# fernandezdaniel/MOBOCMF

Measured on AMD Instinct MI355X. Metric: ELBO steps/sec (MFDGP d=8 M=512 N=8192 S=8), higher is better.
Workload: dtype f64

## Files before the change

mobocmf_amd/csrc/elementwise.hip:

```cpp
#include "common.h"

#define LOG_2PI 1.8378770664093454835606594728112

__device__ __forceinline__ double wave_sum(double v) {
    v += __shfl_xor(v, 1);
    v += __shfl_xor(v, 2);
    v += __shfl_xor(v, 4);
    v += __shfl_xor(v, 8);
    v += __shfl_xor(v, 16);
    v += __shfl_xor(v, 32);
    return v;
}

__device__ __forceinline__ double block_sum(double v, double* sh) {
    v = wave_sum(v);
    const int lane = threadIdx.x & 63, wave = threadIdx.x >> 6;
    __syncthreads();
    if (lane == 0) sh[wave] = v;
    __syncthreads();
    double t = 0.0;
    if (threadIdx.x == 0)
        for (int w = 0; w < (int)(blockDim.x >> 6); ++w) t += sh[w];
    return t;
}
// ... 12 lines not shown

#define GRID1(n) dim3((unsigned)(((n) + 255) / 256)), dim3(256)
#define CHECK_LAUNCH() (hipGetLastError() == hipSuccess ? MOBOCMF_OK : MOBOCMF_HIP_ERROR)

__global__ void zero32_kernel(uint32_t* p, int64_t n) {
    int64_t i = (int64_t)blockIdx.x * blockDim.x + threadIdx.x;
    if (i < n) p[i] = 0u;
}
int launch_zero32(void* ptr, int64_t nwords, hipStream_t s) {
    if (nwords <= 0) return MOBOCMF_OK;
    hipLaunchKernelGGL(zero32_kernel, GRID1(nwords), 0, s, (uint32_t*)ptr, nwords);
    return CHECK_LAUNCH();
}
#define GRIDZ(n, nz) dim3((unsigned)(((n) + 255) / 256), 1, (unsigned)(nz)), dim3(256)
struct ScalZ { const double* p[MAX_ZL]; };
__global__ void zero32_z_kernel(uint32_t* p, int64_t n, int64_t zs_words) {
    int64_t i = (int64_t)blockIdx.x * blockDim.x + threadIdx.x;
    if (i < n) p[blockIdx.z * zs_words + i] = 0u;
}
int launch_zero32_z(void* ptr, int64_t nwords, int nz, int64_t zs_bytes, hipStream_t s) {
    if (nwords <= 0) return MOBOCMF_OK;
    hipLaunchKernelGGL(zero32_z_kernel, GRIDZ(nwords, nz), 0, s, (uint32_t*)ptr, nwords, zs_bytes / 4);
    return CHECK_LAUNCH();
}

__global__ void pad_tril_kernel(const double* src, int64_t lds, int M, double* dst, int Mp) {
    int64_t idx = (int64_t)blockIdx.x * blockDim.x + threadIdx.x;
    if (idx >= (int64_t)Mp * Mp) return;
    int i = (int)(idx / Mp), j = (int)(idx % Mp);
    dst[idx] = (i < M && j <= i) ? src[(int64_t)i * lds + j] : 0.0;
}
int launch_pad_tril(const double* src, int64_t lds, int M, double* dst, int Mp, hipStream_t s) {
    hipLaunchKernelGGL(pad_tril_kernel, GRID1((int64_t)Mp * Mp), 0, s, src, lds, M, dst, Mp);
    return CHECK_LAUNCH();
}

__global__ void pad_vec_kernel(const double* src, int64_t n, double* dst, int64_t np) {
    int64_t i = (int64_t)blockIdx.x * blockDim.x + threadIdx.x;
    if (i < np) dst[i] = (src && i < n) ? src[i] : 0.0;
}
int launch_pad_vec(const double* src, int64_t n, double* dst, int64_t np, hipStream_t s) {
    hipLaunchKernelGGL(pad_vec_kernel, GRID1(np), 0, s, src, n, dst, np);
    return CHECK_LAUNCH();
}

struct PadZ { const double* LS[MAX_ZL]; const double* m[MAX_ZL]; };
__global__ void pad_params_z_kernel(PadZ t, int M, double* LSp, double* mp, int Mp, int64_t zs) {
    int64_t idx = (int64_t)blockIdx.x * blockDim.x + threadIdx.x;
    if (idx >= (int64_t)Mp * Mp) return;
    const int z = blockIdx.z;
    int i = (int)(idx / Mp), j = (int)(idx % Mp);
    LSp[z * zs + idx] = (i < M && j <= i) ? t.LS[z][(int64_t)i * M + j] : 0.0;
    if (idx < Mp) mp[z * zs + idx] = idx < M ? t.m[z][idx] : 0.0;
}
int launch_pad_params_z(const double* const* LS, const double* const* m, int M, double* LSp, double* mp, int Mp, int nz,
                        int64_t zs, hipStream_t s) {
    PadZ t = {};
    for (int z = 0; z < nz; ++z) { t.LS[z] = LS[z]; t.m[z] = m[z]; }
    hipLaunchKernelGGL(pad_params_z_kernel, GRIDZ((int64_t)Mp * Mp, nz), 0, s, t, M, LSp, mp, Mp, zs);
    return CHECK_LAUNCH();
}

__global__ void transpose_kernel(const double* in, int64_t ldi, double* out, int64_t ldo, int64_t rows, int64_t cols,
                                 int64_t zs) {
    __shared__ double t[32][33];
    in += blockIdx.z * zs;
    out += blockIdx.z * zs;
    int64_t c = (int64_t)blockIdx.x * 32 + threadIdx.x, r0 = (int64_t)blockIdx.y * 32;
    for (int k = threadIdx.y; k < 32; k += 8)
        if (r0 + k < rows && c < cols) t[k][threadIdx.x] = in[(r0 + k) * ldi + c];
    __syncthreads();
    int64_t r = r0 + threadIdx.x, c0 = (int64_t)blockIdx.x * 32;
    for (int k = threadIdx.y; k < 32; k += 8)
        if (c0 + k < cols && r < rows) out[(c0 + k) * ldo + r] = t[threadIdx.x][k];
}
int launch_transpose_z(const double* in, int64_t ldi, double* out, int64_t ldo, int64_t rows, int64_t cols, int nz,
                       int64_t zs, hipStream_t s) {
    dim3 grid((unsigned)((cols + 31) / 32), (unsigned)((rows + 31) / 32), (unsigned)nz);
    hipLaunchKernelGGL(transpose_kernel, grid, dim3(32, 8), 0, s, in, ldi, out, ldo, rows, cols, zs);
    return CHECK_LAUNCH();
}
__global__ void transpose_pad_z_kernel(const double* in, double* out, int Mp, int64_t zs, PadZ t, int M, double* LSp, double* mp) {
    __shared__ double tl[32][33];
    const int z = blockIdx.z;
    in += z * zs; out += z * zs;
    const int64_t c = (int64_t)blockIdx.x * 32 + threadIdx.x, r0 = (int64_t)blockIdx.y * 32;
    for (int k = threadIdx.y; k < 32; k += 8) {
        const int64_t i = r0 + k;
        tl[k][threadIdx.x] = in[i * Mp + c];
        LSp[z * zs + i * Mp + c] = (i < M && c <= i) ? t.LS[z][i * M + c] : 0.0;
        if (i == 0) mp[z * zs + c] = c < M ? t.m[z][c] : 0.0;
    }
    __syncthreads();
    const int64_t r = r0 + threadIdx.x, c0 = (int64_t)blockIdx.x * 32;
    for (int k = threadIdx.y; k < 32; k += 8) out[(c0 + k) * Mp + r] = tl[threadIdx.x][k];
}
int launch_transpose_pad_z(const double* in, double* out, int Mp, const double* const* LS, const double* const* m, int M,
                           double* LSp, double* mp, int nz, int64_t zs, hipStream_t s) {
    PadZ t = {};
    for (int z = 0; z < nz; ++z) { t.LS[z] = LS[z]; t.m[z] = m[z]; }
    hipLaunchKernelGGL(transpose_pad_z_kernel, dim3((unsigned)(Mp / 32), (unsigned)(Mp / 32), (unsigned)nz), dim3(32, 8), 0, s, in,
                       out, Mp, zs, t, M, LSp, mp);
    return CHECK_LAUNCH();
}
__global__ void transpose_gemv_z_kernel(const double* in, double* out, int Mp, int64_t zs, const double* Mat, const double* vec,
                                        double* vout) {
    __shared__ double tl[32][33];
    const int z = blockIdx.z;
    in += z * zs; out += z * zs; Mat += z * zs; vec += z * zs; vout += z * zs;
    const int64_t c = (int64_t)blockIdx.x * 32 + threadIdx.x, r0 = (int64_t)blockIdx.y * 32;
    for (int k = threadIdx.y; k < 32; k += 8) tl[k][threadIdx.x] = in[(r0 + k) * Mp + c];
    {
        const int tid = threadIdx.y * 32 + threadIdx.x, wave = tid >> 6, lane = tid & 63;
        const int nblk = gridDim.x * gridDim.y, b = blockIdx.y * gridDim.x + blockIdx.x;
        for (int row = 4 * b + wave; row < Mp; row += 4 * nblk) {
            const double* p = Mat + (int64_t)row * Mp;
            double sacc = 0.0;
            for (int j = lane; j < Mp; j += 64) sacc += p[j] * vec[j];
            sacc = wave_sum(sacc);
            if (lane == 0) vout[row] = sacc;
        }
    }
    __syncthreads();
    const int64_t r = r0 + threadIdx.x, c0 = (int64_t)blockIdx.x * 32;
    for (int k = threadIdx.y; k < 32; k += 8) out[(c0 + k) * Mp + r] = tl[threadIdx.x][k];
}
int launch_transpose_gemv_z(const double* in, double* out, int Mp, const double* Mat, const double* vec, double* vout, int nz,
                            int64_t zs, hipStream_t s) {
    hipLaunchKernelGGL(transpose_gemv_z_kernel, dim3((unsigned)(Mp / 32), (unsigned)(Mp / 32), (unsigned)nz), dim3(32, 8), 0, s, in,
                       out, Mp, zs, Mat, vec, vout);
    return CHECK_LAUNCH();
}
int launch_transpose(const double* in, int64_t ldi, double* out, int64_t ldo, int64_t rows, int64_t cols, hipStream_t s) {
    return launch_transpose_z(in, ldi, out, ldo, rows, cols, 1, 0, s);
}

__global__ void gemv_rows_kernel(const double* Mat, int64_t ld, const double* vec, double* out, int rows, int64_t cols,
                                 double scale, int accumulate, int64_t zs) {
    int row = blockIdx.x * 4 + (threadIdx.x >> 6);
    int lane = threadIdx.x & 63;
    if (row >= rows) return;
    Mat += blockIdx.z * zs; vec += blockIdx.z * zs; out += blockIdx.z * zs;
    const double* p = Mat + (int64_t)row * ld;
    double s = 0.0;
    for (int64_t j = lane; j < cols; j += 64) s += p[j] * vec[j];
    s = wave_sum(s) * scale;
    if (lane == 0) out[row] = accumulate ? out[row] + s : s;
}
int launch_gemv_rows_z(const double* Mat, int64_t ld, const double* vec, double* out, int rows, int64_t cols, double scale,
                       int accumulate, int nz, int64_t zs, hipStream_t s) {
    hipLaunchKernelGGL(gemv_rows_kernel, dim3((rows + 3) / 4, 1, nz), dim3(256), 0, s, Mat, ld, vec, out, rows, cols, scale,
                       accumulate, zs);
    return CHECK_LAUNCH();
}
int launch_gemv_rows(const double* Mat, int64_t ld, const double* vec, double* out, int rows, int64_t cols, double scale,
                     int accumulate, hipStream_t s) {
    return launch_gemv_rows_z(Mat, ld, vec, out, rows, cols, scale, accumulate, 1, 0, s);
}

__global__ void kl_part_kernel(const double* L, const double* LSp, const double* U, const double* a, int M, int Mp,
                               double* part, int64_t zs) {
    __shared__ double sh[4];
    double s = 0.0;
    const int r0 = blockIdx.x * 4;
    L += blockIdx.z * zs; LSp += blockIdx.z * zs; U += blockIdx.z * zs; a += blockIdx.z * zs; part += blockIdx.z * zs;
    for (int rr = 0; rr < 4; ++rr) {
        const int i = r0 + rr;
        if (i >= M) break;
        const double* u = U + (int64_t)i * Mp;
        for (int j = threadIdx.x; j <= i; j += 256) s += u[j] * u[j];
        if (threadIdx.x == 0) {
            double l = L[(int64_t)i * Mp + i], ls = LSp[(int64_t)i * Mp + i];
            s += 2.0 * log(l) - log(ls * ls) + a[i] * a[i];
        }
    }
    s = block_sum(s, sh);
    if (threadIdx.x == 0) part[blockIdx.x] = s;
}
struct KlZ { double* p[MAX_ZL]; };
__global__ void kl_final_kernel(const double* part, int np, int M, KlZ kl, int64_t zs) {
    __shared__ double sh[4];
    double s = 0.0;
    part += blockIdx.x * zs;
    for (int i = threadIdx.x; i < np; i += 256) s += part[i];
    s = block_sum(s, sh);
    if (threadIdx.x == 0) kl.p[blockIdx.x][0] = 0.5 * (s - (double)M);
}
__global__ __launch_bounds__(1024) void kl_one_kernel(const double* L, const double* LSp, const double* U, const double* a, int M,
                                                      int Mp, KlZ kl, int64_t zs) {
    __shared__ double sh[16];
    const int z = blockIdx.x;
    L += z * zs; LSp += z * zs; U += z * zs; a += z * zs;
    double s = 0.0;
    const int total = M * Mp;
#pragma unroll 4
    for (int e = threadIdx.x; e < total; e += 1024) {
        const int i = e / Mp, j = e - i * Mp;
        const double u = U[e];
        s += j <= i ? u * u : 0.0;
    }
    for (int i = threadIdx.x; i < M; i += 1024) {
        const double l = L[(int64_t)i * Mp + i], ls = LSp[(int64_t)i * Mp + i];
        s += 2.0 * log(l) - log(ls * ls) + a[i] * a[i];
    }
    s = wave_sum(s);
    if ((threadIdx.x & 63) == 0) sh[threadIdx.x >> 6] = s;
    __syncthreads();
    if (threadIdx.x == 0) {
        double t = 0.0;
        for (int w = 0; w < 16; ++w) t += sh[w];
        kl.p[z][0] = 0.5 * (t - (double)M);
    }
}
int launch_kl_z(const double* L, const double* LSp, const double* U, const double* a, int M, int Mp, double* const* kl,
                double* part, int nz, int64_t zs, hipStream_t s) {
    if (M <= 128) {
        KlZ kz1 = {};
        for (int z = 0; z < nz; ++z) kz1.p[z] = kl[z];
        hipLaunchKernelGGL(kl_one_kernel, dim3(nz), dim3(1024), 0, s, L, LSp, U, a, M, Mp, kz1, zs);
        return CHECK_LAUNCH();
    }
    const int nb = (M + 3) / 4;
    hipLaunchKernelGGL(kl_part_kernel, dim3(nb, 1, nz), dim3(256), 0, s, L, LSp, U, a, M, Mp, part, zs);
    KlZ kz = {};
    for (int z = 0; z < nz; ++z) kz.p[z] = kl[z];
    hipLaunchKernelGGL(kl_final_kernel, dim3(nz), dim3(256), 0, s, (const double*)part, nb, M, kz, zs);
    return CHECK_LAUNCH();
}
int launch_kl(const double* L, const double* LSp, const double* U, const double* a, int M, int Mp, double* kl,
              double* part, hipStream_t s) {
    double* one[1] = {kl};
    return launch_kl_z(L, LSp, U, a, M, Mp, one, part, 1, 0, s);
}

__global__ void moments_finish_kernel(const double* qpart, const double* mupart, const double* rpart, int nrb,
                                      int64_t Np, int64_t N, const double* knn, int branch, double min_var, double* q,
                                      double* r, double* varraw, double* mean, double* var, int32_t* zero_word) {
    int64_t n = (int64_t)blockIdx.x * blockDim.x + threadIdx.x;
    if (n == 0 && zero_word) zero_word[0] = 0;
    if (n >= Np) return;
    double qs = 0, ms = 0, rs = 0;
    for (int b = 0; b < nrb; ++b) {
        qs += qpart[(int64_t)b * Np + n];
        ms += mupart[(int64_t)b * Np + n];
        rs += rpart[(int64_t)b * Np + n];
    }
    double sres = knn[n] - qs;
    if (!branch && sres < 0.0) sres = 0.0;
    double v = sres + rs;
    q[n] = qs;
    r[n] = rs;
    varraw[n] = v;
    if (n < N) {
        mean[n] = ms;
        var[n] = v < min_var ? min_var : v;
    }
}
int launch_moments_finish(const double* qpart, const double* mupart, const double* rpart, int nrb, int64_t Np, int64_t N,
                          const double* knn, int branch, double min_var, double* q, double* r, double* varraw,
                          double* mean, double* var, int32_t* zero_word, hipStream_t s) {
    hipLaunchKernelGGL(moments_finish_kernel, GRID1(Np), 0, s, qpart, mupart, rpart, nrb, Np, N, knn, branch, min_var, q,
                       r, varraw, mean, var, zero_word);
    return CHECK_LAUNCH();
}

__global__ void moments_bwd_prep_kernel(const double* g_mean, const double* g_var, const double* knn, const double* q,
                                        const double* varraw, int branch, double min_var, int64_t N, int64_t Np,
                                        double* gmu, double* gv, double* gv2, double* cgv, int32_t* nclamped, int32_t* blkact) {
    __shared__ int any_w[4];
    int64_t n = (int64_t)blockIdx.x * blockDim.x + threadIdx.x;
    double gm = 0.0, g = 0.0, c = 0.0;
    if (n < N) {
        gm = g_mean ? g_mean[n] : 0.0;
        g = (g_var && varraw[n] > min_var) ? g_var[n] : 0.0;
        c = (branch || knn[n] - q[n] > 0.0) ? g : 0.0;
        if (c != g) atomicAdd(nclamped, 1);
    }
    if (n < Np) {
        gmu[n] = gm;
        gv[n] = g;
        gv2[n] = 2.0 * g;
        cgv[n] = c;
    }
    if (blkact) {
        const bool any = !(gm == 0.0) || !(g == 0.0);
        const unsigned long long b = __ballot(any);
        if ((threadIdx.x & 63) == 0) any_w[threadIdx.x >> 6] = b != 0ull ? 1 : 0;
        __syncthreads();
        if (threadIdx.x < 2) {
            const int64_t blk = (int64_t)blockIdx.x * 2 + threadIdx.x;
            if (blk * 128 < Np) blkact[blk] = any_w[2 * threadIdx.x] | any_w[2 * threadIdx.x + 1];
        }
    }
}
int launch_moments_bwd_prep(const double* g_mean, const double* g_var, const double* knn, const double* q,
                            const double* varraw, int branch, double min_var, int64_t N, int64_t Np, double* gmu,
                            double* gv, double* gv2, double* cgv, int32_t* nclamped, int zeroed, int32_t* blkact, hipStream_t s) {
    if (!zeroed && launch_zero32(nclamped, 1, s)) return MOBOCMF_HIP_ERROR;
    hipLaunchKernelGGL(moments_bwd_prep_kernel, GRID1(Np), 0, s, g_mean, g_var, knn, q, varraw, branch, min_var, N, Np,
                       gmu, gv, gv2, cgv, nclamped, blkact);
    return CHECK_LAUNCH();
}

__device__ __forceinline__ double slab_sum(const double* p, int64_t slab_stride, int ns) {
    double v = 0.0;
    int z = 0;
    for (; z + 8 <= ns; z += 8) {
        double t[8];
#pragma unroll
        for (int b = 0; b < 8; ++b) t[b] = p[(z + b) * slab_stride];
#pragma unroll
        for (int b = 0; b < 8; ++b) v += t[b];
    }
    for (; z < ns; ++z) v += p[z * slab_stride];
    return v;
}

__global__ void reduce_slabs_sym_kernel(const double* slabs, int64_t slab_stride, int nslab, int nslab_diag, double* out,
                                        int Mp, const int32_t* flag, const double* fallback) {
    int64_t idx = (int64_t)blockIdx.x * blockDim.x + threadIdx.x;
    if (idx >= (int64_t)Mp * Mp) return;
    int i = (int)(idx / Mp), j = (int)(idx % Mp);
    if (flag && *flag == 0) {
        out[idx] = fallback[idx];
        return;
    }
    if (j / TILE > i / TILE) return;
    const double* p = j > i ? slabs + (int64_t)j * Mp + i : slabs + (int64_t)i * Mp + j;
    const int ns = (i / TILE == j / TILE) ? nslab_diag : nslab;
    const double v = slab_sum(p, slab_stride, ns);
    out[idx] = v;
    if (j / TILE < i / TILE) out[(int64_t)j * Mp + i] = v;
}
__global__ void reduce_slabs_sym2_kernel(const double* slabs, const double* slabs2, int64_t slab_stride, int nslab,
                                         int nslab_diag, double* out, double* out2, int Mp, const int32_t* flag) {
    int64_t idx = (int64_t)blockIdx.x * blockDim.x + threadIdx.x;
    if (idx >= (int64_t)Mp * Mp) return;
    int i = (int)(idx / Mp), j = (int)(idx % Mp);
    if (j / TILE > i / TILE) return;
    const int64_t off = j > i ? (int64_t)j * Mp + i : (int64_t)i * Mp + j;
    const int ns = (i / TILE == j / TILE) ? nslab_diag : nslab;
    const double v = slab_sum(slabs + off, slab_stride, ns);
    double v2 = v;
    if (*flag != 0) v2 = slab_sum(slabs2 + off, slab_stride, ns);
    out[idx] = v;
    out2[idx] = v2;
    if (j / TILE < i / TILE) { out[(int64_t)j * Mp + i] = v; out2[(int64_t)j * Mp + i] = v2; }
}
int launch_reduce_slabs_sym2(const double* slabs, const double* slabs2, int64_t slab_stride, int nslab, int nslab_diag,
                             double* out, double* out2, int Mp, const int32_t* flag, hipStream_t s) {
    hipLaunchKernelGGL(reduce_slabs_sym2_kernel, GRID1((int64_t)Mp * Mp), 0, s, slabs, slabs2, slab_stride, nslab, nslab_diag,
                       out, out2, Mp, flag);
    return CHECK_LAUNCH();
}
int launch_reduce_slabs_sym(const double* slabs, int64_t slab_stride, int nslab, int nslab_diag, double* out, int Mp,
                            const int32_t* flag, const double* fallback, hipStream_t s) {
    hipLaunchKernelGGL(reduce_slabs_sym_kernel, GRID1((int64_t)Mp * Mp), 0, s, slabs, slab_stride, nslab, nslab_diag, out, Mp,
                       flag, fallback);
    return CHECK_LAUNCH();
}

__global__ void dutot_y_kernel(const double* G1, const double* G2, const double* Hc, const double* U, const double* da,
                               const double* a, ScalZ gklz, int Mp, double* dU, double* da_tot, double* Y, int64_t zs) {
    __shared__ double tl[32][33];
    const double* gkl = gklz.p[blockIdx.z];
    const double g = gkl ? gkl[0] : 0.0;
    const int64_t zo = blockIdx.z * zs;
    G1 += zo; G2 += zo; Hc += zo; U += zo; da += zo; a += zo; dU += zo; da_tot += zo; Y += zo;
    const int nt = Mp / 32, ti = blockIdx.x / nt, tj = blockIdx.x % nt;
    const int tx = threadIdx.x & 31, ty = threadIdx.x >> 5;
    if (tj <= ti) {
#pragma unroll
        for (int r = ty; r < 32; r += 8) tl[r][tx] = G1[(int64_t)(tj * 32 + r) * Mp + ti * 32 + tx];
    }
    __syncthreads();
#pragma unroll
    for (int r = ty; r < 32; r += 8) {
        const int i = ti * 32 + r, j = tj * 32 + tx;
        const int64_t idx = (int64_t)i * Mp + j;
        const double ai = a[i], aj = a[j], dai = da[i], daj = da[j];
        dU[idx] = j <= i ? 2.0 * tl[tx][r] + g * U[idx] : 0.0;
        Y[idx] = 2.0 * (G2[idx] - Hc[idx]) + ai * daj + (dai + g * ai) * aj;
        if (tj == 0 && tx == 0) da_tot[i] = dai + g * ai;
    }
}
int launch_dutot_y_z(const double* G1, const double* G2, const double* Hc, const double* U, const double* da, const double* a,
                     const double* const* gkl, int Mp, double* dU, double* da_tot, double* Y, int nz, int64_t zs, hipStream_t s) {
    ScalZ t = {};
    for (int z = 0; z < nz; ++z) t.p[z] = gkl[z];
    const int nt = Mp / 32;
    hipLaunchKernelGGL(dutot_y_kernel, dim3((unsigned)(nt * nt), 1, (unsigned)nz), dim3(256), 0, s, G1, G2, Hc, U, da, a, t, Mp,
                       dU, da_tot, Y, zs);
    return CHECK_LAUNCH();
}


__global__ void add_kl_terms_kernel(double* dU, const double* U, double* da, const double* a, const double* gkl, int Mp) {
    int64_t idx = (int64_t)blockIdx.x * blockDim.x + threadIdx.x;
    const double g = gkl ? gkl[0] : 0.0;
    if (idx < (int64_t)Mp * Mp) dU[idx] += g * U[idx];
    if (idx < Mp) da[idx] += g * a[idx];
}
int launch_add_kl_terms(double* dU, const double* U, double* da, const double* a, const double* gkl, int Mp, hipStream_t s) {
    hipLaunchKernelGGL(add_kl_terms_kernel, GRID1((int64_t)Mp * Mp), 0, s, dU, U, da, a, gkl, Mp);
    return CHECK_LAUNCH();
}

__global__ void rank1_add_kernel(double* X, const double* u, const double* v, int Mp) {
    int64_t idx = (int64_t)blockIdx.x * blockDim.x + threadIdx.x;
    if (idx >= (int64_t)Mp * Mp) return;
    int i = (int)(idx / Mp), j = (int)(idx % Mp);
    X[idx] += u[i] * v[j];
}
int launch_rank1_add(double* X, const double* u, const double* v, int Mp, hipStream_t s) {
    hipLaunchKernelGGL(rank1_add_kernel, GRID1((int64_t)Mp * Mp), 0, s, X, u, v, Mp);
    return CHECK_LAUNCH();
}

__global__ void dl_from_t2_kernel(const double* T2, const double* L, ScalZ gklz, int M, int Mp, double* dL, int64_t zs) {
    int64_t idx = (int64_t)blockIdx.x * blockDim.x + threadIdx.x;
    if (idx >= (int64_t)Mp * Mp) return;
    const double* gkl = gklz.p[blockIdx.z];
    T2 += blockIdx.z * zs; L += blockIdx.z * zs; dL += blockIdx.z * zs;
    int i = (int)(idx / Mp), j = (int)(idx % Mp);
    double v = 0.0;
    if (i < M && j <= i) {
        v = -T2[idx];
        if (i == j && gkl) v += gkl[0] / L[idx];
    }
    dL[idx] = v;
}
int launch_dl_from_t2_z(const double* T2, const double* L, const double* const* gkl, int M, int Mp, double* dL, int nz,
                        int64_t zs, hipStream_t s) {
    ScalZ t = {};
    for (int z = 0; z < nz; ++z) t.p[z] = gkl[z];
    hipLaunchKernelGGL(dl_from_t2_kernel, GRIDZ((int64_t)Mp * Mp, nz), 0, s, T2, L, t, M, Mp, dL, zs);
    return CHECK_LAUNCH();
}
int launch_dl_from_t2(const double* T2, const double* L, const double* gkl, int M, int Mp, double* dL, hipStream_t s) {
    const double* one[1] = {gkl};
    return launch_dl_from_t2_z(T2, L, one, M, Mp, dL, 1, 0, s);
}

__global__ void phi_kernel(const double* T3, int Mp, double* P, int64_t zs) {
    int64_t idx = (int64_t)blockIdx.x * blockDim.x + threadIdx.x;
    if (idx >= (int64_t)Mp * Mp) return;
    T3 += blockIdx.z * zs; P += blockIdx.z * zs;
    int i = (int)(idx / Mp), j = (int)(idx % Mp);
    P[idx] = j < i ? T3[idx] : (j == i ? 0.5 * T3[idx] : 0.0);
}
int launch_phi_z(const double* T3, int Mp, double* P, int nz, int64_t zs, hipStream_t s) {
    hipLaunchKernelGGL(phi_kernel, GRIDZ((int64_t)Mp * Mp, nz), 0, s, T3, Mp, P, zs);
    return CHECK_LAUNCH();
}
int launch_phi(const double* T3, int Mp, double* P, hipStream_t s) { return launch_phi_z(T3, Mp, P, 1, 0, s); }

__global__ void symmetrize_kernel(const double* S, int Mp, double* G, int64_t zs) {
    int64_t idx = (int64_t)blockIdx.x * blockDim.x + threadIdx.x;
    if (idx >= (int64_t)Mp * Mp) return;
    S += blockIdx.z * zs; G += blockIdx.z * zs;
    int i = (int)(idx / Mp), j = (int)(idx % Mp);
    G[idx] = 0.5 * (S[idx] + S[(int64_t)j * Mp + i]);
}
int launch_symmetrize_z(const double* S, int Mp, double* G, int nz, int64_t zs, hipStream_t s) {
    hipLaunchKernelGGL(symmetrize_kernel, GRIDZ((int64_t)Mp * Mp, nz), 0, s, S, Mp, G, zs);
    return CHECK_LAUNCH();
}
int launch_symmetrize(const double* S, int Mp, double* G, hipStream_t s) { return launch_symmetrize_z(S, Mp, G, 1, 0, s); }

__global__ void gls_out_kernel(const double* X, const double* LSp, const double* gkl, int M, int Mp, double* gLS) {
    int64_t idx = (int64_t)blockIdx.x * blockDim.x + threadIdx.x;
    if (idx >= (int64_t)M * M) return;
    int i = (int)(idx / M), j = (int)(idx % M);
    double v = 0.0;
    if (j <= i) {
        v = X[(int64_t)i * Mp + j];
        if (i == j && gkl) v -= gkl[0] / LSp[(int64_t)i * Mp + i];
    }
    gLS[idx] = v;
}
int launch_gls_out(const double* X, const double* LSp, const double* gkl, int M, int Mp, double* gLS, hipStream_t s) {
    hipLaunchKernelGGL(gls_out_kernel, GRID1((int64_t)M * M), 0, s, X, LSp, gkl, M, Mp, gLS);
    return CHECK_LAUNCH();
}

struct ChainOutZ { const double* gkl[MAX_ZL]; double* gLS[MAX_ZL]; double* gm[MAX_ZL]; };
__global__ void chain_outputs_z_kernel(const double* X, const double* LSp, const double* LinvT, const double* da_tot, int M,
                                       int Mp, ChainOutZ t, int nb_ls, int64_t zs) {
    const int z = blockIdx.y;
    X += z * zs; LSp += z * zs; LinvT += z * zs; da_tot += z * zs;
    if ((int)blockIdx.x < nb_ls) {
        const int64_t idx = (int64_t)blockIdx.x * blockDim.x + threadIdx.x;
        if (idx >= (int64_t)M * M) return;
        const int i = (int)(idx / M), j = (int)(idx % M);
        double v = 0.0;
        if (j <= i) {
            v = X[(int64_t)i * Mp + j];
            if (i == j && t.gkl[z]) v -= t.gkl[z][0] / LSp[(int64_t)i * Mp + i];
        }
        t.gLS[z][idx] = v;
        return;
    }
    const int row = ((int)blockIdx.x - nb_ls) * 4 + (threadIdx.x >> 6), lane = threadIdx.x & 63;
    if (row >= M) return;
    const double* p = LinvT + (int64_t)row * Mp;
    double sacc = 0.0;
    for (int j = lane; j < Mp; j += 64) sacc += p[j] * da_tot[j];
    sacc = wave_sum(sacc);
    if (lane == 0) t.gm[z][row] = sacc;
}
int launch_chain_outputs_z(const double* X, const double* LSp, const double* LinvT, const double* da_tot, int M, int Mp,
                           const double* const* gkl, double* const* gLS, double* const* gm, int nz, int64_t zs, hipStream_t s) {
    ChainOutZ t = {};
    for (int z = 0; z < nz; ++z) { t.gkl[z] = gkl[z]; t.gLS[z] = gLS[z]; t.gm[z] = gm[z]; }
    const int nb_ls = (int)(((int64_t)M * M + 255) / 256), nb_m = (M + 3) / 4;
    hipLaunchKernelGGL(chain_outputs_z_kernel, dim3((unsigned)(nb_ls + nb_m), (unsigned)nz), dim3(256), 0, s, X, LSp, LinvT, da_tot,
                       M, Mp, t, nb_ls, zs);
    return CHECK_LAUNCH();
}

__global__ void copy_block_kernel(const double* src, int64_t lds, double* dst, int64_t ldd, int64_t rows, int64_t cols) {
    int64_t idx = (int64_t)blockIdx.x * blockDim.x + threadIdx.x;
    if (idx >= rows * cols) return;
    int64_t i = idx / cols, j = idx % cols;
    dst[i * ldd + j] = src[i * lds + j];
}
int launch_copy_block(const double* src, int64_t lds, double* dst, int64_t ldd, int64_t rows, int64_t cols, hipStream_t s) {
    hipLaunchKernelGGL(copy_block_kernel, GRID1(rows * cols), 0, s, src, lds, dst, ldd, rows, cols);
    return CHECK_LAUNCH();
}

__global__ __launch_bounds__(256) void mirror_lower_kernel(const double* src, int64_t lds_, double* dst, int64_t ldd,
                                                           int64_t row0, int64_t rows, int64_t cols, int64_t n_real) {
    __shared__ double t[32][33];
    const int64_t ti = blockIdx.y, tj = blockIdx.x;
    if (tj > ti) return;
    const int tx = threadIdx.x & 31, ty = threadIdx.x >> 5;
    for (int r = ty; r < 32; r += 8) {
        const int64_t i = ti * 32 + r, j = tj * 32 + tx;
        double v = 0.0;
        if (i < rows && j < cols) v = src[i * lds_ + j];
        t[r][tx] = v;
        if (i >= j && row0 + i < n_real && row0 + j < n_real && j < cols) dst[(row0 + i) * ldd + row0 + j] = v;
    }
    __syncthreads();
    for (int r = ty; r < 32; r += 8) {
        const int64_t j = tj * 32 + r, i = ti * 32 + tx;
        if (i > j && row0 + i < n_real && row0 + j < n_real && j < cols && i < rows) dst[(row0 + j) * ldd + row0 + i] = t[tx][r];
    }
}
int launch_mirror_lower(const double* src, int64_t lds_, double* dst, int64_t ldd, int64_t row0, int64_t rows, int64_t cols,
                        int64_t n_real, hipStream_t s) {
    const dim3 grid((unsigned)((cols + 31) / 32), (unsigned)((rows + 31) / 32));
    hipLaunchKernelGGL(mirror_lower_kernel, grid, dim3(256), 0, s, src, lds_, dst, ldd, row0, rows, cols, n_real);
    return CHECK_LAUNCH();
}

__global__ void mf_combine_kernel(const double* Ks, const double* Kn, int64_t ld, const double* s1, const double* s2,
                                  const int32_t* l1, const int32_t* l2, const double* ntab, int64_t n1, int64_t n2,
                                  double diag, double* out, int64_t ldo, int64_t rows_p, int64_t cols_p) {
    const int64_t idx = (int64_t)blockIdx.x * blockDim.x + threadIdx.x;
    if (idx >= rows_p * cols_p) return;
    const int64_t i = idx / cols_p, j = idx % cols_p;
    double v = 0.0;
    if (i < n1 && j < n2) {
        const int a = l1[i], b = l2[j];
        v = (s1 ? s1[i] : 1.0) * (s2 ? s2[j] : 1.0) * Ks[i * ld + j] + ntab[a < b ? a : b] * Kn[i * ld + j];
        if (i == j) v += diag;
    } else if (i == j && diag != 0.0) {
        v = 1.0;
    }
    out[i * ldo + j] = v;
}
int launch_mf_combine(const double* Ks, const double* Kn, int64_t ld, const double* s1, const double* s2, const int32_t* l1,
                      const int32_t* l2, const double* ntab, int64_t n1, int64_t n2, double diag, double* out, int64_t ldo,
                      int64_t rows_p, int64_t cols_p, hipStream_t s) {
    hipLaunchKernelGGL(mf_combine_kernel, GRID1(rows_p * cols_p), 0, s, Ks, Kn, ld, s1, s2, l1, l2, ntab, n1, n2, diag, out,
                       ldo, rows_p, cols_p);
    return CHECK_LAUNCH();
}
__global__ void copy_pad_identity_kernel(const double* src, int64_t lds_, int n, double* dst, int np) {
    const int64_t idx = (int64_t)blockIdx.x * blockDim.x + threadIdx.x;
    if (idx >= (int64_t)np * np) return;
    const int i = (int)(idx / np), j = (int)(idx % np);
    dst[idx] = (i < n && j < n) ? src[(int64_t)i * lds_ + j] : (i == j ? 1.0 : 0.0);
}
int launch_copy_pad_identity(const double* src, int64_t lds_, int n, double* dst, int np, hipStream_t s) {
    hipLaunchKernelGGL(copy_pad_identity_kernel, GRID1((int64_t)np * np), 0, s, src, lds_, n, dst, np);
    return CHECK_LAUNCH();
}
__global__ void exact_gp_mll_kernel(const double* L, int64_t ld, const double* a, int n, double* mll) {
    __shared__ double sh[4];
    double s = 0.0;
    for (int i = threadIdx.x; i < n; i += blockDim.x) s += -0.5 * a[i] * a[i] - log(L[(int64_t)i * ld + i]);
    s = block_sum(s, sh);
    if (threadIdx.x == 0) mll[0] = s - 0.5 * n * 1.8378770664093453;
}
int launch_exact_gp_mll(const double* L, int64_t ld, const double* a, int n, double* mll, hipStream_t s) {
    hipLaunchKernelGGL(exact_gp_mll_kernel, dim3(1), dim3(256), 0, s, L, ld, a, n, mll);
    return CHECK_LAUNCH();
}
__global__ void exact_gp_finish_kernel(const double* qpart, const double* mupart, int nparts, int64_t ntp, int64_t nt,
                                       const double* kss, double* mean, double* var) {
    const int64_t j = (int64_t)blockIdx.x * blockDim.x + threadIdx.x;
    if (j >= nt) return;
    double q = 0.0, m = 0.0;
    for (int p = 0; p < nparts; ++p) { q += qpart[(int64_t)p * ntp + j]; m += mupart[(int64_t)p * ntp + j]; }
    mean[j] = m;
    var[j] = kss[j] - q;
}
int launch_exact_gp_finish(const double* qpart, const double* mupart, int nparts, int64_t ntp, int64_t nt, const double* kss,
                           double* mean, double* var, hipStream_t s) {
    hipLaunchKernelGGL(exact_gp_finish_kernel, GRID1(nt), 0, s, qpart, mupart, nparts, ntp, nt, kss, mean, var);
    return CHECK_LAUNCH();
}

__global__ void propagate_fwd_kernel(const double* mean, const double* var, const double* eps, double* f, int64_t n,
                                     int div) {
    int64_t i = (int64_t)blockIdx.x * blockDim.x + threadIdx.x;
    if (i >= n) return;
    int64_t b = i / div;
    f[i] = mean[b] + sqrt(var[b]) * eps[i];
}
__global__ void propagate_rng_fwd_kernel(const double* mean, const double* var, int64_t* rng_state, double* f, double* eps_out,
                                         int64_t n, int div) {
    const uint64_t seed = (uint64_t)rng_state[0], call = (uint64_t)__atomic_load_n(&rng_state[1], __ATOMIC_RELAXED);
    const int64_t i = (int64_t)blockIdx.x * blockDim.x + threadIdx.x;
    if (i < n) {
        const int64_t b = i / div;
        const double e = philox_normal(seed, call, (uint64_t)i);
        eps_out[i] = e;
        f[i] = mean[b] + sqrt(var[b]) * e;
    }
    __syncthreads();
    if (threadIdx.x == 0) {
        const unsigned long long t = atomicAdd((unsigned long long*)&rng_state[2], 1ull);
        if (t == (unsigned long long)gridDim.x - 1) {
            __atomic_store_n(&rng_state[2], (int64_t)0, __ATOMIC_RELAXED);
            __atomic_store_n(&rng_state[1], (int64_t)(call + 1), __ATOMIC_RELAXED);
        }
    }
}
__global__ void propagate_bwd_kernel(const double* var, const double* eps, const double* gf, double* gmean, double* gvar,
                                     int64_t nbase, int div, int64_t nprev, const double* add_mean, const double* add_var) {
    int64_t b = (int64_t)blockIdx.x * blockDim.x + threadIdx.x;
    if (b >= nprev) return;
    const double am = add_mean ? add_mean[b] : 0.0, av = add_var ? add_var[b] : 0.0;
    if (b >= nbase) {
        gmean[b] = am;
        gvar[b] = av;
        return;
    }
    double sm = 0.0, sv = 0.0;
    for (int s = 0; s < div; ++s) {
        double g = gf[b * div + s];
        sm += g;
        sv += g * eps[b * div + s];
    }
    gmean[b] = sm + am;
    gvar[b] = sv * 0.5 / sqrt(var[b]) + av;
// ... 828 lines not shown
```

Measured before the change: 1054.

## Reduce symmetric slab sums over lower-triangle strips with vector loads and transposed stores

```diff
diff --git a/mobocmf_amd/csrc/elementwise.hip b/mobocmf_amd/csrc/elementwise.hip
--- a/mobocmf_amd/csrc/elementwise.hip
+++ b/mobocmf_amd/csrc/elementwise.hip
@@ -338,60 +338,112 @@
     return CHECK_LAUNCH();
 }
 
-__device__ __forceinline__ double slab_sum(const double* p, int64_t slab_stride, int ns) {
-    double v = 0.0;
+#define RS_ROWS 8
+#define RS_COLS 64
+#define RS_LD (RS_COLS + 2)
+#define RS_PER_TILE ((TILE / RS_ROWS) * (TILE / RS_COLS))
+typedef double rs_v2 __attribute__((ext_vector_type(2)));
+
+struct SymStrip { int rb, cb, r0, c0; };
+__device__ __forceinline__ SymStrip sym_strip_of_block() {
+    const int t = (int)blockIdx.x / RS_PER_TILE, q = (int)blockIdx.x % RS_PER_TILE;
+    SymStrip S;
+    int r = 0;
+    while ((r + 1) * (r + 2) / 2 <= t) ++r;
+    S.rb = r;
+    S.cb = t - r * (r + 1) / 2;
+    S.r0 = (q >> 1) * RS_ROWS;
+    S.c0 = (q & 1) * RS_COLS;
+    return S;
+}
+__device__ __forceinline__ rs_v2 sym_strip_sum(const double* slabs, int64_t slab_stride, int ns, int Mp, const SymStrip& S) {
+    const int tid = threadIdx.x;
+    const double* p = slabs + ((int64_t)S.rb * TILE + S.r0 + (tid >> 5)) * Mp + (int64_t)S.cb * TILE + S.c0 + 2 * (tid & 31);
+    rs_v2 v = (rs_v2){0.0, 0.0};
     int z = 0;
-    for (; z + 8 <= ns; z += 8) {
-        double t[8];
+    for (; z + 16 <= ns; z += 16) {
+        rs_v2 t[16];
 #pragma unroll
-        for (int b = 0; b < 8; ++b) t[b] = p[(z + b) * slab_stride];
+        for (int b = 0; b < 16; ++b) t[b] = *(const rs_v2*)(p + (z + b) * slab_stride);
 #pragma unroll
-        for (int b = 0; b < 8; ++b) v += t[b];
-    }
-    for (; z < ns; ++z) v += p[z * slab_stride];
+        for (int b = 0; b < 16; ++b) v += t[b];
+    }
+    for (; z + 4 <= ns; z += 4) {
+        rs_v2 t[4];
+#pragma unroll
+        for (int b = 0; b < 4; ++b) t[b] = *(const rs_v2*)(p + (z + b) * slab_stride);
+#pragma unroll
+        for (int b = 0; b < 4; ++b) v += t[b];
+    }
+    for (; z < ns; ++z) v += *(const rs_v2*)(p + z * slab_stride);
     return v;
 }
-
-__global__ void reduce_slabs_sym_kernel(const double* slabs, int64_t slab_stride, int nslab, int nslab_diag, double* out,
-                                        int Mp, const int32_t* flag, const double* fallback) {
-    int64_t idx = (int64_t)blockIdx.x * blockDim.x + threadIdx.x;
-    if (idx >= (int64_t)Mp * Mp) return;
-    int i = (int)(idx / Mp), j = (int)(idx % Mp);
+__device__ __forceinline__ void sym_strip_store(rs_v2 v, double* out, int Mp, const SymStrip& S, double* st) {
+    const int tid = threadIdx.x;
+    const bool diag = S.rb == S.cb;
+    {
+        const int r = S.r0 + (tid >> 5), c = S.c0 + 2 * (tid & 31);
+        double* o = out + ((int64_t)S.rb * TILE + r) * Mp + (int64_t)S.cb * TILE + c;
+        if (!diag) *(rs_v2*)o = v;
+        else {
+            if (c <= r) o[0] = v[0];
+            if (c + 1 <= r) o[1] = v[1];
+        }
+        st[(tid >> 5) * RS_LD + 2 * (tid & 31)] = v[0];
+        st[(tid >> 5) * RS_LD + 2 * (tid & 31) + 1] = v[1];
+    }
+    __syncthreads();
+    const int j = tid >> 2, h = tid & 3;
+    const double m0 = st[(2 * h) * RS_LD + j], m1 = st[(2 * h + 1) * RS_LD + j];
+    double* o = out + ((int64_t)S.cb * TILE + S.c0 + j) * Mp + (int64_t)S.rb * TILE + S.r0 + 2 * h;
+    if (!diag) *(rs_v2*)o = (rs_v2){m0, m1};
+    else {
+        if (S.c0 + j < S.r0 + 2 * h) o[0] = m0;
+        if (S.c0 + j < S.r0 + 2 * h + 1) o[1] = m1;
+    }
+    __syncthreads();
+}
+__global__ __launch_bounds__(256) void reduce_slabs_sym_kernel(const double* slabs, int64_t slab_stride, int nslab, int nslab_diag,
+                                                               double* out, int Mp, const int32_t* flag, const double* fallback) {
+    __shared__ double st[RS_ROWS * RS_LD];
+    const SymStrip S = sym_strip_of_block();
+    if (S.rb == S.cb && S.c0 > S.r0 + RS_ROWS - 1) return;
     if (flag && *flag == 0) {
-        out[idx] = fallback[idx];
+        for (int e = threadIdx.x; e < RS_ROWS * RS_COLS; e += 256) {
+            const int64_t i = (int64_t)S.rb * TILE + S.r0 + e / RS_COLS, jj = (int64_t)S.cb * TILE + S.c0 + e % RS_COLS;
+            if (jj <= i) out[i * Mp + jj] = fallback[i * Mp + jj];
+            if (jj < i) out[jj * Mp + i] = fallback[jj * Mp + i];
+        }
         return;
     }
-    if (j / TILE > i / TILE) return;
-    const double* p = j > i ? slabs + (int64_t)j * Mp + i : slabs + (int64_t)i * Mp + j;
-    const int ns = (i / TILE == j / TILE) ? nslab_diag : nslab;
-    const double v = slab_sum(p, slab_stride, ns);
-    out[idx] = v;
-    if (j / TILE < i / TILE) out[(int64_t)j * Mp + i] = v;
-}
-__global__ void reduce_slabs_sym2_kernel(const double* slabs, const double* slabs2, int64_t slab_stride, int nslab,
-                                         int nslab_diag, double* out, double* out2, int Mp, const int32_t* flag) {
-    int64_t idx = (int64_t)blockIdx.x * blockDim.x + threadIdx.x;
-    if (idx >= (int64_t)Mp * Mp) return;
-    int i = (int)(idx / Mp), j = (int)(idx % Mp);
-    if (j / TILE > i / TILE) return;
-    const int64_t off = j > i ? (int64_t)j * Mp + i : (int64_t)i * Mp + j;
-    const int ns = (i / TILE == j / TILE) ? nslab_diag : nslab;
-    const double v = slab_sum(slabs + off, slab_stride, ns);
-    double v2 = v;
-    if (*flag != 0) v2 = slab_sum(slabs2 + off, slab_stride, ns);
-    out[idx] = v;
-    out2[idx] = v2;
-    if (j / TILE < i / TILE) { out[(int64_t)j * Mp + i] = v; out2[(int64_t)j * Mp + i] = v2; }
+    const rs_v2 v = sym_strip_sum(slabs, slab_stride, S.rb == S.cb ? nslab_diag : nslab, Mp, S);
+    sym_strip_store(v, out, Mp, S, st);
+}
+__global__ __launch_bounds__(256) void reduce_slabs_sym2_kernel(const double* slabs, const double* slabs2, int64_t slab_stride,
+                                                                int nslab, int nslab_diag, double* out, double* out2, int Mp,
+                                                                const int32_t* flag) {
+    __shared__ double st[RS_ROWS * RS_LD];
+    const SymStrip S = sym_strip_of_block();
+    if (S.rb == S.cb && S.c0 > S.r0 + RS_ROWS - 1) return;
+    const int ns = S.rb == S.cb ? nslab_diag : nslab;
+    rs_v2 v = sym_strip_sum(slabs, slab_stride, ns, Mp, S);
+    sym_strip_store(v, out, Mp, S, st);
+    if (*flag != 0) v = sym_strip_sum(slabs2, slab_stride, ns, Mp, S);
+    sym_strip_store(v, out2, Mp, S, st);
+}
+static dim3 sym_strip_grid(int Mp) {
+    const int nrb = Mp / TILE;
+    return dim3((unsigned)(nrb * (nrb + 1) / 2 * RS_PER_TILE));
 }
 int launch_reduce_slabs_sym2(const double* slabs, const double* slabs2, int64_t slab_stride, int nslab, int nslab_diag,
                              double* out, double* out2, int Mp, const int32_t* flag, hipStream_t s) {
-    hipLaunchKernelGGL(reduce_slabs_sym2_kernel, GRID1((int64_t)Mp * Mp), 0, s, slabs, slabs2, slab_stride, nslab, nslab_diag,
+    hipLaunchKernelGGL(reduce_slabs_sym2_kernel, sym_strip_grid(Mp), dim3(256), 0, s, slabs, slabs2, slab_stride, nslab, nslab_diag,
                        out, out2, Mp, flag);
     return CHECK_LAUNCH();
 }
 int launch_reduce_slabs_sym(const double* slabs, int64_t slab_stride, int nslab, int nslab_diag, double* out, int Mp,
                             const int32_t* flag, const double* fallback, hipStream_t s) {
-    hipLaunchKernelGGL(reduce_slabs_sym_kernel, GRID1((int64_t)Mp * Mp), 0, s, slabs, slab_stride, nslab, nslab_diag, out, Mp,
+    hipLaunchKernelGGL(reduce_slabs_sym_kernel, sym_strip_grid(Mp), dim3(256), 0, s, slabs, slab_stride, nslab, nslab_diag, out, Mp,
                        flag, fallback);
     return CHECK_LAUNCH();
 }
```

Result: no change. 1061 (median of 6 runs) (+0.7%).
